# alshai/pfbwt-f

Measured on AMD Instinct MI355X. Metric: Gbases/s end-to-end BWT+SA build; bit-exact .bwt/.sa vs reference, higher is better.
Workload: dtype u8 text / u32 indices / u64 hash; 1 GPU; S-32G; L=32000000, H=1000, seed=1000, w=10, p=100, flags=-r, uint_t=64, n=32000010000, r=83625322, input=text resident in HBM, outputs (.bwt, .ssa, .esa) left in HBM, per_rank=single GPU

## Files before the change

pfbwt-f_amd/csrc/emit.h:

```cpp
#pragma once
#include "prims.h"
#include "parse.h"

namespace pfp {

__global__ __launch_bounds__(BLOCK) void k_pbwt_pack(const uint32_t *P, const uint8_t *last, const tpos_t *sai, uint64_t m, uint4 *rec)
{
    const uint64_t j = (uint64_t)blockIdx.x * BLOCK + threadIdx.x;
    if (j >= m) return;
    const uint64_t v = sai ? (uint64_t)sai[j] : 0ULL;
    rec[j] = make_uint4((uint32_t)v, (uint32_t)(v >> 32), P[j], (uint32_t)last[j ? j - 1 : m - 1]);
}
constexpr int BWL_SHIFT = 29;
__device__ __forceinline__ uint32_t bwl_code(uint32_t c) { return c == 0 ? 0u : c == Dollar ? 1u : c == '-' ? 2u : c == 'A' ? 3u : c == 'C' ? 4u : c == 'G' ? 5u : c == 'N' ? 6u : c == 'T' ? 7u : 8u; }
__device__ __forceinline__ uint8_t bwl_byte(uint32_t code) { return code == 0 ? (uint8_t)0 : code == 1 ? Dollar : code == 2 ? (uint8_t)'-' : code == 3 ? (uint8_t)'A' : code == 4 ? (uint8_t)'C' : code == 5 ? (uint8_t)'G' : code == 6 ? (uint8_t)'N' : (uint8_t)'T'; }
__global__ __launch_bounds__(BLOCK) void k_pbwt_rows(const uint32_t *SAP, const uint4 *rec, uint64_t m, uint8_t *bwlast, tpos_t *bwsai, uint32_t *W, uint32_t *rowid, int pack, uint32_t *bad)
{
    const uint64_t i = (uint64_t)blockIdx.x * BLOCK + threadIdx.x;
    if (i > m) return;
    const uint32_t s = SAP[i];
    if (s == 0) { bwlast[i] = 0; if (bwsai) bwsai[i] = 0; W[i] = 0; rowid[i] = (uint32_t)i; return; }
    const uint4 R = rec[s - 1];
    bwlast[i] = (uint8_t)R.w;
    if (bwsai) bwsai[i] = (tpos_t)(((uint64_t)R.y << 32) | R.x);
// ... 626 lines not shown

constexpr int EG_BUF = 4096, EG_PER_THREAD = EG_BUF / BLOCK;
constexpr int EG1_BUF = 8192, EG2_BUF = 16384;
__device__ __forceinline__ uint32_t group_members(const EmitArgs &a, const uint4 &S) { const uint32_t k = S.w & 0xFFFFFFu; return k == 0xFFFFFFu ? a.gk[S.z] : k; }
template <typename EBT> __global__ __launch_bounds__(BLOCK) void k_special_pack(EmitArgs a, uint32_t nsp, uint4 *cinfo, unsigned long long *cgb)
{
    const uint64_t j = (uint64_t)blockIdx.x * BLOCK + threadIdx.x;
    if (j >= nsp) return;
    const uint32_t i = a.elist[j]; const uint4 S = a.sinfo[i];
    const uint32_t fl = S.w >> 24; const bool multi = (fl & SF_MULTI) != 0;
    cinfo[j] = make_uint4(S.x, multi ? group_members(a, S) : 1u, multi ? i - S.z : 0u, (uint32_t)a.s_pc[i] | (fl << 8));
    cgb[j] = (unsigned long long)reinterpret_cast<const EBT *>(a.EB)[multi ? S.z : i];
}
template <typename EBT> __device__ __forceinline__ uint64_t group_start_at_or_after(const EBT *ENB, const uint4 *cinfo, uint64_t nsp, uint64_t lo, uint64_t v)
{
    while (lo < nsp && (uint64_t)ENB[lo] < v) ++lo;
    if (lo >= nsp) return nsp;
    const uint4 ci = cinfo[lo];
    if (!((ci.w >> 8) & SF_MULTI)) return lo;
    const uint64_t head = lo - ci.z;
    return (uint64_t)ENB[head] < v ? head + ci.y : head;
}
template <typename EBT> __global__ __launch_bounds__(BLOCK) void k_tile_own(const EBT *ENB, const uint4 *cinfo, const uint32_t *etile_slot, uint64_t nsp, uint64_t ntiles, uint32_t *town)
{
    const uint64_t t = (uint64_t)blockIdx.x * BLOCK + threadIdx.x;
    if (t > ntiles) return;
    town[t] = (uint32_t)group_start_at_or_after<EBT>(ENB, cinfo, nsp, etile_slot[t], t * EMIT_TILE);
}
template <typename EBT> __global__ __launch_bounds__(BLOCK) void k_emit_groups(EmitArgs a, uint8_t *bwt, uint32_t *qrow)
{
    __shared__ uint32_t LQ[EG_BUF];
    __shared__ uint32_t s_eb[EG_SLOTS + 1], s_fb[EG_SLOTS], s_kf[EG_SLOTS], s_dl[EG_SLOTS];
    __shared__ uint64_t s_ob[EG_SLOTS];
    __shared__ uint8_t s_pc[EG_SLOTS];
    __shared__ uint32_t red[4];
    __shared__ uint64_t jb[2];
    const EBT *ENB = reinterpret_cast<const EBT *>(a.ENB);
    const uint64_t tile0 = a.e0 / EMIT_TILE, tb = tile0 + blockIdx.x;
    const uint64_t o0 = tb * EMIT_TILE > a.e0 ? tb * EMIT_TILE : a.e0;
    const uint64_t o1 = ((tb + 1) * EMIT_TILE < a.e1) ? (tb + 1) * EMIT_TILE : a.e1;
    if (threadIdx.x < 2) {
        const uint64_t v = threadIdx.x ? o1 : o0;
        const uint64_t tv = threadIdx.x ? tb + 1 : tb;
        uint64_t j;
        if (v == tv * EMIT_TILE) j = a.town[tv];
        else {
            uint64_t lo = a.etile_slot[tb], hi = (uint64_t)a.etile_slot[tb + 1] + 1u;
            if (hi > a.ecount) hi = a.ecount;
            if (lo > hi) lo = hi;
            while (lo < hi) { const uint64_t mid = lo + ((hi - lo) >> 1); if ((uint64_t)ENB[mid] < v) lo = mid + 1; else hi = mid; }
            j = group_start_at_or_after<EBT>(ENB, a.cinfo, a.ecount, lo, v);
        }
        jb[threadIdx.x] = j;
    }
    __syncthreads();
    uint64_t j = jb[0]; const uint64_t jE = jb[1];
    const uint32_t cap = a.group_rows_cap < (uint32_t)EG_BUF ? a.group_rows_cap : (uint32_t)EG_BUF;
    while (j < jE) {
        const uint32_t nload = jE - j < (uint64_t)EG_SLOTS ? (uint32_t)(jE - j) : (uint32_t)EG_SLOTS;
        const uint64_t B0 = (uint64_t)ENB[j];
        uint32_t cand[2] = {0u, 0u}, bad = 0xFFFFFFFFu;
#pragma unroll
        for (int t = 0; t < 2; ++t) {
            const uint32_t s = threadIdx.x + (uint32_t)t * BLOCK;
            if (s < nload) {
                const uint4 ci = a.cinfo[j + s];
                const uint32_t fl = ci.w >> 8, dl = ci.z, k = ci.y;
                const uint64_t e0 = (uint64_t)ENB[j + s] - B0, e1 = (uint64_t)ENB[j + s + 1] - B0;
                s_eb[s] = e0 < 0xFFFFFFFFull ? (uint32_t)e0 : 0xFFFFFFFFu;
                if (s + 1 == nload) s_eb[nload] = e1 < 0xFFFFFFFFull ? (uint32_t)e1 : 0xFFFFFFFFu;
                s_fb[s] = ci.x; s_kf[s] = (k < 0xFFFFFFu ? k : 0xFFFFFFu) | (fl << 24); s_dl[s] = dl; s_pc[s] = (uint8_t)ci.w;
                s_ob[s] = (uint64_t)a.cgb[j + s];
                if (((fl & (SF_GFULL | SF_BIG)) || k > a.rank_members_max) && s < bad) bad = s;
                if (dl + 1u == k && e1 <= (uint64_t)cap) cand[t] = s + 1u;
            }
        }
        uint32_t tot;
        (void)block_incl_max(~bad, red, &tot);
        const uint32_t firstbad = ~tot;
        uint32_t c = 0;
#pragma unroll
        for (int t = 0; t < 2; ++t) if (cand[t] && cand[t] <= firstbad && cand[t] > c) c = cand[t];
        uint32_t cut;
        (void)block_incl_max(c, red, &cut);
        if (cut == 0) {
            const uint32_t k0 = a.cinfo[j].y;
            const uint64_t r0 = B0, r1 = (uint64_t)ENB[j + k0];
            {
                const uint32_t f0 = s_kf[0] >> 24;
                if (threadIdx.x == 0) {
                    unsigned long long idx = ~0ULL;
                    if (a.lglist && (f0 & SF_MULTI) && !(f0 & (SF_GFULL | SF_BIG)) && k0 <= (uint32_t)EG_SLOTS && r1 - r0 <= (uint64_t)EG2_BUF) {
                        const int big = r1 - r0 > (uint64_t)EG1_BUF ? 1 : 0;
                        idx = atomicAdd(a.lgcount + big, 1ULL);
                        if (idx < a.lgcap) a.lglist[(uint64_t)big * a.lgcap + idx] = (uint32_t)j;
                    }
                    jb[0] = idx < a.lgcap ? 1 : 0;
                }
                __syncthreads();
                const bool taken = jb[0] != 0;
                __syncthreads();
                if (taken) { j += k0; continue; }
            }
            if (threadIdx.x == 0) a.gleft[j] = 1;
            if (a.gstat && threadIdx.x == 0) {
                const uint32_t f0 = s_kf[0] >> 24;
                atomicAdd(&a.gstat[(f0 & SF_GFULL) ? 0 : (f0 & SF_BIG) ? 1 : (r1 - r0 > (uint64_t)cap) ? 2 : 3], (unsigned long long)(r1 - r0));
                int b = 0; while (b < 7 && (1024ull << (2 * b)) <= r1 - r0) ++b;
                atomicAdd(&a.gstat[4 + b], (unsigned long long)(r1 - r0));
            }
            if (r1 > r0) for (uint64_t t = r0 / EMIT_TILE + threadIdx.x; t <= (r1 - 1) / EMIT_TILE; t += BLOCK) a.tile_left[t - tile0] = 1;
            j += k0;
            __syncthreads();
            continue;
        }
        __syncthreads();
        const uint32_t nrows = s_eb[cut];
#pragma unroll
        for (int t = 0; t < 2; ++t) { const uint32_t s = threadIdx.x + (uint32_t)t * BLOCK; if (s < cut) s_ob[s] -= (uint64_t)s_eb[s - s_dl[s]]; }
        uint32_t qv[EG_PER_THREAD], sv[EG_PER_THREAD]; uint8_t cv[EG_PER_THREAD];
#pragma unroll
        for (int it = 0; it < EG_PER_THREAD; ++it) {
            const uint32_t r = threadIdx.x + (uint32_t)it * BLOCK;
            sv[it] = 0; qv[it] = 0; cv[it] = 0;
            if (r < nrows) {
                const uint32_t s = upper_bound_t<uint32_t>(s_eb, cut, r) - 1u, at = s_fb[s] + (r - s_eb[s]);
                sv[it] = s; qv[it] = a.ilist[at];
                if (!((s_kf[s] >> 24) & SF_MULTI) && a.bwl_il) cv[it] = a.bwl_il[at];
            }
        }
#pragma unroll
        for (int it = 0; it < EG_PER_THREAD; ++it) {
            const uint32_t r = threadIdx.x + (uint32_t)it * BLOCK;
            if (r < nrows) { LQ[r] = qv[it]; const uint32_t fl = s_kf[sv[it]] >> 24; if (fl & SF_MULTI) cv[it] = s_pc[sv[it]]; else if (!a.bwl_il) cv[it] = a.bwlast[qv[it]]; }
        }
        __syncthreads();
#pragma unroll
        for (int it = 0; it < EG_PER_THREAD; ++it) {
            const uint32_t r = threadIdx.x + (uint32_t)it * BLOCK;
            if (r < nrows) {
                const uint32_t s = sv[it], kf = s_kf[s];
                uint32_t pos = r;
                if ((kf >> 24) & SF_MULTI) {
                    const uint32_t sh = s - s_dl[s], k = kf & 0xFFFFFFu, q = qv[it];
                    uint32_t before = 0;
                    for (uint32_t mm = 0; mm < k; ++mm) {
                        const uint32_t sm = sh + mm;
                        if (sm != s) before += lower_bound_u32(LQ + s_eb[sm], s_eb[sm + 1] - s_eb[sm], q);
                    }
                    pos = s_eb[sh] + before + (r - s_eb[s]);
                }
                if (qrow) qrow[B0 - a.q0 + pos] = qv[it];
                const uint64_t o = s_ob[s] + pos;
                if (o >= a.w0 && o < a.w1) bwt[o - a.w0] = cv[it];
            }
        }
        __syncthreads();
        j += cut;
    }
}

template <int ITEMS> __device__ __forceinline__ void lds_sort_pairs_u32(uint32_t *keys, uint16_t *vals, uint32_t n, int npass, uint32_t (*wh)[RS_RADIX], uint32_t *red)
{
    const int lane = threadIdx.x & 63, wave = threadIdx.x >> 6;
    const uint32_t nit = (n + BLOCK - 1) / BLOCK;
    for (uint32_t j = n + threadIdx.x; j < nit * BLOCK; j += BLOCK) { keys[j] = 0xFFFFFFFFu; vals[j] = 0; }
    const uint32_t base = (uint32_t)wave * (nit * WAVE) + lane;
    for (int p = 0; p < npass; ++p) {
        const int sh = 8 * p;
        uint32_t k[ITEMS], dg[ITEMS]; uint16_t v[ITEMS];
#pragma unroll
        for (int w = 0; w < BLOCK / WAVE; ++w) wh[w][threadIdx.x] = 0;
        __syncthreads();
#pragma unroll
        for (int it = 0; it < ITEMS; ++it) {
            if ((uint32_t)it < nit) {
                const uint32_t i = base + (uint32_t)it * WAVE;
                k[it] = keys[i]; v[it] = vals[i];
                const uint32_t d = (k[it] >> sh) & 255u;
                uint32_t plo = 0xFFFFFFFFu, phi = 0xFFFFFFFFu;
                same_digit_lanes(d, plo, phi);
                const int leader = plo ? __builtin_ctz(plo) : 32 + __builtin_ctz(phi);
                uint32_t old = 0;
                if (lane == leader) { old = wh[wave][d]; wh[wave][d] = old + (uint32_t)__builtin_popcount(plo) + (uint32_t)__builtin_popcount(phi); }
                old = __shfl(old, leader);
                dg[it] = d | ((old + __builtin_amdgcn_mbcnt_hi(phi, __builtin_amdgcn_mbcnt_lo(plo, 0u))) << 8);
            }
        }
        __syncthreads();
        {
            const unsigned d = threadIdx.x;
            uint32_t cw[BLOCK / WAVE]; uint32_t total = 0;
#pragma unroll
            for (int w = 0; w < BLOCK / WAVE; ++w) { cw[w] = wh[w][d]; total += cw[w]; }
            uint32_t tt;
            uint32_t run = block_excl_sum(total, red, &tt);
#pragma unroll
            for (int w = 0; w < BLOCK / WAVE; ++w) { wh[w][d] = run; run += cw[w]; }
        }
        __syncthreads();
#pragma unroll
        for (int it = 0; it < ITEMS; ++it) {
            if ((uint32_t)it < nit) { const uint32_t li = wh[wave][dg[it] & 255u] + (dg[it] >> 8); keys[li] = k[it]; vals[li] = v[it]; }
        }
        __syncthreads();
    }
}
template <typename EBT, int BUF> __global__ __launch_bounds__(BLOCK) void k_emit_groups_large(EmitArgs a, uint8_t *bwt, uint32_t *qrow)
{
    __shared__ uint32_t LQ[BUF];
    __shared__ uint16_t LS[BUF];
    __shared__ uint32_t wh[BLOCK / WAVE][RS_RADIX];
    __shared__ uint32_t s_eb[EG_SLOTS + 1], s_fb[EG_SLOTS];
    __shared__ uint8_t s_pc[EG_SLOTS];
    __shared__ uint32_t red[4];
    const EBT *ENB = reinterpret_cast<const EBT *>(a.ENB);
    constexpr int WHICH = BUF > EG1_BUF ? 1 : 0;
    const unsigned long long have = a.lgcount[WHICH];
    const uint64_t cnt = have < a.lgcap ? have : a.lgcap;
    for (uint64_t g = blockIdx.x; g < cnt; g += gridDim.x) {
        const uint64_t j = a.lglist[(uint64_t)WHICH * a.lgcap + g];
        const uint32_t k = a.cinfo[j].y;
        const uint64_t B0 = (uint64_t)ENB[j], outbase = (uint64_t)a.cgb[j];
        for (uint32_t s = threadIdx.x; s < k; s += BLOCK) {
            const uint4 ci = a.cinfo[j + s];
            s_eb[s] = (uint32_t)((uint64_t)ENB[j + s] - B0); s_fb[s] = ci.x; s_pc[s] = (uint8_t)ci.w;
            if (s + 1 == k) s_eb[k] = (uint32_t)((uint64_t)ENB[j + k] - B0);
        }
        __syncthreads();
        const uint32_t nrows = s_eb[k];
        for (uint32_t r = threadIdx.x; r < nrows; r += BLOCK) { const uint32_t s = upper_bound_t<uint32_t>(s_eb, k, r) - 1u; LQ[r] = a.ilist[s_fb[s] + (r - s_eb[s])]; LS[r] = (uint16_t)s; }
        __syncthreads();
        lds_sort_pairs_u32<BUF / BLOCK>(LQ, LS, nrows, a.qpasses, wh, red);
        for (uint32_t r = threadIdx.x; r < nrows; r += BLOCK) {
            if (qrow) qrow[B0 - a.q0 + r] = LQ[r];
            const uint64_t o = outbase + r;
            if (o >= a.w0 && o < a.w1) bwt[o - a.w0] = s_pc[LS[r]];
        }
        __syncthreads();
    }
}

template <typename EBT> __global__ __launch_bounds__(BLOCK) void k_slice_bounds(EmitArgs a, uint64_t lo, uint64_t hi, unsigned long long *out)
{
    if (blockIdx.x != 0 || threadIdx.x != 0) return;
    const EBT *EB = reinterpret_cast<const EBT *>(a.EB);
    const EBT *ENB = reinterpret_cast<const EBT *>(a.ENB);
    const uint32_t il = slot_of_row<EBT>(a, lo);
    const uint32_t gh = (a.s_fl[il] & SF_MULTI) ? a.s_g0[il] : il;
    out[0] = EB[gh];
    out[2] = a.special ? (unsigned long long)ENB[a.cpos[gh]] : 0ULL;
    if (hi >= a.nout) { out[1] = a.nout; out[3] = a.special ? (unsigned long long)ENB[a.ecount] : 0ULL; return; }
    uint32_t s = slot_of_row<EBT>(a, hi - 1);
    if (a.s_fl[s] & SF_MULTI) { const uint32_t g = a.s_g0[s]; while (s < a.dsize && (a.s_fl[s] & SF_MULTI) && a.s_g0[s] == g) ++s; }
    else ++s;
    {
        uint64_t lo_ = s, hi_ = a.dsize;
        while (lo_ < hi_) { const uint64_t mid = lo_ + ((hi_ - lo_) >> 1); if ((uint64_t)EB[mid] < hi) lo_ = mid + 1; else hi_ = mid; }
        s = (uint32_t)lo_;
    }
    out[1] = s < a.dsize ? (uint64_t)EB[s] : a.nout;
    out[3] = a.special ? (unsigned long long)ENB[s < a.dsize ? a.cpos[s] : a.ecount] : 0ULL;
}

#ifndef PFP_FILL_NT
#define PFP_FILL_NT 0
#endif
__device__ __forceinline__ void fill_store16(uint8_t *dst, uint32_t x0, uint32_t x1, uint32_t x2, uint32_t x3)
{
#if PFP_FILL_NT && !defined(PFBWT_EMU_HIP_RUNTIME_H)
    typedef uint32_t fill_v4u __attribute__((ext_vector_type(4)));
    fill_v4u v = {x0, x1, x2, x3};
    __builtin_nontemporal_store(v, reinterpret_cast<fill_v4u *>(dst));
#else
    *reinterpret_cast<uint4 *>(dst) = make_uint4(x0, x1, x2, x3);
#endif
}
constexpr int FILL_PER_THREAD = 16, FILL_SUB = BLOCK * FILL_PER_THREAD;
constexpr int FILL_GROUPS = 4;
constexpr uint32_t FILL_MAX_SUBS = 8;
static_assert(FILL_SUB % EMIT_TILE == 0, "fill tiles are whole emission tiles");
template <typename EBT> __global__ __launch_bounds__(BLOCK) void k_fill(EmitArgs a, uint8_t *bwt, uint32_t subs_per_wg)
{
    __shared__ uint32_t eb[FILL_SUB + 2];
    __shared__ uint8_t pcs[FILL_SUB + 2];
    __shared__ uint32_t wcnt[BLOCK / WAVE];
    __shared__ uint32_t sts[FILL_MAX_SUBS * FILL_GROUPS + 1];
    const EBT *EB = reinterpret_cast<const EBT *>(a.EB);
    const EBT *cnt = reinterpret_cast<const EBT *>(a.cnt);
    const uint64_t ntiles = (a.nout + EMIT_TILE - 1) / EMIT_TILE;
    constexpr uint64_t TPS = FILL_SUB / EMIT_TILE;
    constexpr uint64_t SUPER = (uint64_t)FILL_GROUPS * FILL_SUB;
    const uint64_t st0 = a.w0 / SUPER + (uint64_t)blockIdx.x * subs_per_wg;
    const int lane = threadIdx.x & 63, wave = threadIdx.x >> 6;
    const unsigned long long lt = lane ? (~0ULL >> (64 - lane)) : 0ULL;
    for (uint32_t k = threadIdx.x; k <= subs_per_wg * FILL_GROUPS; k += BLOCK) {
        const uint64_t t = (st0 * FILL_GROUPS + k) * TPS;
        sts[k] = a.tile_slot[t < ntiles ? t : ntiles];
    }
    __syncthreads();
    auto compact = [&](uint32_t i0, uint32_t i1, uint64_t base) -> uint32_t {
        const uint32_t ns = i1 - i0 + 1u;
        uint32_t nz = 0;
        for (uint32_t k0 = 0; k0 < ns; k0 += BLOCK) {
            const uint32_t k = k0 + threadIdx.x;
            const EBT cn = k < ns ? cnt[i0 + k] : (EBT)0;
            const uint64_t e = k < ns ? (uint64_t)EB[i0 + k] : 0ULL;
            const uint8_t pc = k < ns ? a.s_pc[i0 + k] : (uint8_t)0;
            const bool has = cn != 0;
            const unsigned long long bal = __ballot(has);
            __syncthreads();
            if (lane == 0) wcnt[wave] = (uint32_t)__popcll(bal);
            __syncthreads();
            uint32_t pos = nz, tot = 0;
#pragma unroll
            for (int v = 0; v < BLOCK / WAVE; ++v) { const uint32_t cw = wcnt[v]; if (v < wave) pos += cw; tot += cw; }
            if (nz + tot > (uint32_t)FILL_SUB + 1u) return ~0u;
            if (has) { pos += (uint32_t)__popcll(bal & lt); eb[pos] = e > base ? (uint32_t)(e - base) : 0u; pcs[pos] = pc; }
            nz += tot;
        }
        if (threadIdx.x == 0) eb[nz] = 0xFFFFFFFFu;
        __syncthreads();
        return nz;
    };
    auto write_group = [&](uint64_t g0, uint64_t base, uint32_t nz) {
        const uint64_t o0 = g0 > a.w0 ? g0 : a.w0;
        const uint64_t o1 = g0 + FILL_SUB < a.w1 ? g0 + FILL_SUB : a.w1;
        const uint64_t ra = g0 + (uint64_t)threadIdx.x * FILL_PER_THREAD;
        const uint64_t lo = ra > o0 ? ra : o0, hi = ra + FILL_PER_THREAD < o1 ? ra + FILL_PER_THREAD : o1;
        if (lo >= hi) return;
        uint32_t wd[FILL_PER_THREAD / 4] = {0, 0, 0, 0};
        uint32_t rel = (uint32_t)(lo - base);
        uint32_t s = upper_bound_t<uint32_t>(eb, nz, rel) - 1u;
        uint32_t nxt = eb[s + 1], c = pcs[s];
        if (lo == ra && hi == ra + FILL_PER_THREAD && nxt >= rel + FILL_PER_THREAD) {
            wd[0] = wd[1] = wd[2] = wd[3] = c * 0x01010101u;
        } else {
#pragma unroll
            for (int j = 0; j < FILL_PER_THREAD; ++j) {
                const uint64_t o = ra + j;
                if (o >= lo && o < hi) {
                    while (rel >= nxt) { ++s; nxt = eb[s + 1]; c = pcs[s]; }
                    wd[j >> 2] |= c << (8 * (j & 3));
                    ++rel;
                }
            }
        }
        uint8_t *dst = bwt + (ra - a.w0);
        if (lo == ra && hi == ra + FILL_PER_THREAD) fill_store16(dst, wd[0], wd[1], wd[2], wd[3]);
        else for (uint64_t o = lo; o < hi; ++o) { const int j = (int)(o - ra); dst[j] = (uint8_t)(wd[j >> 2] >> (8 * (j & 3))); }
    };
    for (uint32_t ss = 0; ss < subs_per_wg; ++ss) {
        const uint64_t tstart = (st0 + ss) * SUPER;
        if (tstart >= a.w1) break;
        const uint64_t tend = tstart + SUPER < a.w1 ? tstart + SUPER : a.w1;
        const uint32_t ng = (uint32_t)((tend - tstart + FILL_SUB - 1) / FILL_SUB);
        const uint32_t *gs = sts + ss * FILL_GROUPS;
        uint32_t nz = compact(gs[0], gs[ng], tstart);
        if (nz != ~0u) {
            for (uint32_t g = 0; g < ng; ++g) write_group(tstart + (uint64_t)g * FILL_SUB, tstart, nz);
        } else {
            for (uint32_t g = 0; g < ng; ++g) {
                const uint64_t g0 = tstart + (uint64_t)g * FILL_SUB;
                nz = compact(gs[g], gs[g + 1], g0);
                write_group(g0, g0, nz);
            }
        }
    }
}

__global__ __launch_bounds__(BLOCK) void k_run_count(const uint8_t *bwt, uint64_t nout, int has_prev, unsigned long long *runs)
{
    __shared__ uint32_t red[4];
    const uint64_t o0 = ((uint64_t)blockIdx.x * BLOCK + threadIdx.x) * 16;
    uint32_t cntr = 0;
    if (o0 < nout) {
        uint8_t prev = (o0 || has_prev) ? *(bwt + o0 - 1) : (uint8_t)0;
        for (int k = 0; k < 16 && o0 + k < nout; ++k) { const uint8_t cc = bwt[o0 + k]; cntr += cc != prev; prev = cc; }
    }
    uint32_t tot;
    (void)block_excl_sum(cntr, red, &tot);
    if (threadIdx.x == 0 && tot) atomicAdd(runs, (unsigned long long)tot);
}
constexpr int RUN_PER_THREAD = 16, RUN_TILE = BLOCK * RUN_PER_THREAD;
__device__ __forceinline__ uint32_t run_mask16(const uint8_t *bwt, uint64_t j0, uint64_t rows, int has_prev)
{
    if (j0 >= rows) return 0;
    const uint64_t lo = ld8(bwt + j0), hi = ld8(bwt + j0 + 8);
    const uint64_t prev = (j0 || has_prev) ? (uint64_t)*(bwt + j0 - 1) : 0ULL;
    const uint64_t xl = lo ^ ((lo << 8) | prev), xh = hi ^ ((hi << 8) | (lo >> 56));
    uint32_t m = 0;
#pragma unroll
    for (int b = 0; b < 8; ++b) { m |= ((xl >> (8 * b)) & 0xff) ? (1u << b) : 0u; m |= ((xh >> (8 * b)) & 0xff) ? (1u << (8 + b)) : 0u; }
    const uint64_t left = rows - j0;
    return left >= 16 ? m : (m & ((1u << left) - 1u));
}
__global__ __launch_bounds__(BLOCK) void k_run_tile_count(const uint8_t *bwt, uint64_t rows, int has_prev, uint32_t *tilecnt, uint16_t *rmask)
{
    __shared__ uint32_t red[4];
    const uint64_t g = (uint64_t)blockIdx.x * BLOCK + threadIdx.x;
    const uint32_t m = run_mask16(bwt, g * RUN_PER_THREAD, rows, has_prev);
    if (rmask) rmask[g] = (uint16_t)m;
    uint32_t tot;
    (void)block_excl_sum((uint32_t)__popc(m), red, &tot);
    if (threadIdx.x == 0) tilecnt[blockIdx.x] = tot;
}
constexpr int SR_TILES = 8;
template <typename SAT> __global__ __launch_bounds__(BLOCK) void k_sample_rows(const uint16_t *rmask, uint64_t rows, uint64_t ntiles, const uint32_t *tilebase, uint64_t row_base, uint64_t run_base, uint64_t total_rows,
                                                                               uint64_t total_runs_plus1 , SAT *ssa, SAT *esa)
{
    __shared__ unsigned long long red[4];
    const uint64_t t0 = (uint64_t)blockIdx.x * SR_TILES;
    uint32_t m[SR_TILES]; unsigned long long c[2] = {0ULL, 0ULL};
#pragma unroll
    for (int b = 0; b < SR_TILES; ++b) {
        const uint64_t g = (t0 + b) * BLOCK + threadIdx.x;
        m[b] = (t0 + b < ntiles && g * RUN_PER_THREAD < rows) ? (uint32_t)rmask[g] : 0u;
        c[b >> 2] |= (unsigned long long)__popc(m[b]) << (16 * (b & 3));
    }
    unsigned long long tot;
    const unsigned long long e0 = block_excl_sum(c[0], red, &tot), e1 = block_excl_sum(c[1], red, &tot);
#pragma unroll
    for (int b = 0; b < SR_TILES; ++b) {
        if (t0 + b >= ntiles) break;
        const uint64_t j0 = ((t0 + b) * BLOCK + threadIdx.x) * RUN_PER_THREAD;
        uint32_t mm = m[b];
        uint64_t k = run_base + tilebase[t0 + b] + (uint32_t)(((b < 4 ? e0 : e1) >> (16 * (b & 3))) & 0xFFFFu);
        while (mm) {
            const int bit = __ffs((int)mm) - 1; mm &= mm - 1;
            const uint64_t o = row_base + j0 + bit;
            ssa[2 * k] = (SAT)o;
            if (o) esa[2 * (k - 1)] = (SAT)(o - 1);
            ++k;
        }
        if (total_runs_plus1 && j0 < rows && row_base + rows == total_rows && total_rows - 1 - row_base - j0 < RUN_PER_THREAD)
            *(esa + 2 * ((long long)total_runs_plus1 - 2)) = (SAT)(total_rows - 1);
    }
}
template <typename SAT, typename EBT> __global__ __launch_bounds__(BLOCK) void k_sample_values(EmitArgs a, const SAT *sa_win, const uint32_t *qrow, uint64_t w_first, uint64_t rc, uint64_t run_base,
                                                                                               int has_last, uint64_t last_idx, SAT *ssa, SAT *esa)
{
    const EBT *EB = reinterpret_cast<const EBT *>(a.EB);
    auto value = [&](uint64_t o) -> SAT {
        if (sa_win) return sa_win[o - w_first];
        if (o == 0) return (SAT)a.n;
        const uint32_t slot = slot_of_row<EBT>(a, o);
        uint32_t q;
        if (!a.special) q = qrow[o - w_first];
        else {
            const uint4 S = a.sinfo[slot]; const uint32_t fl = S.w >> 24;
            if (slot_is_special(fl)) {
                const uint32_t g = (fl & SF_MULTI) ? S.z : slot;
                q = a.qspec[(uint64_t)reinterpret_cast<const EBT *>(a.ENB)[a.cpos[g]] - a.q0 + (o - (uint64_t)EB[g])];
            } else if (!(fl & SF_MULTI)) q = a.ilist[S.x + (uint32_t)(o - (uint64_t)EB[slot])];
            else q = (o == (uint64_t)EB[S.z]) ? a.gqf[S.z] : a.gql[S.z];
        }
        return (SAT)((SAT)a.bwsai[q] - (SAT)a.s_sl[slot]);
    };
    const uint64_t i = (uint64_t)blockIdx.x * BLOCK + threadIdx.x;
    if (i < rc) {
        const uint64_t k = run_base + i;
        const uint64_t o = (uint64_t)ssa[2 * k];
        ssa[2 * k + 1] = value(o);
        if (o) esa[2 * (k - 1) + 1] = value(o - 1);
    } else if (i == rc && has_last) *(esa + 2 * (long long)last_idx + 1) = value(a.nout - 1);
}

}
```

Before: 124.2 Gbases/s.

## Prefetch compaction loads, hint run search, fill runs wordwise, compact whole workgroup span

The BWT fill kernel now software-prefetches the next block's count/boundary/char loads during compaction. It keeps a per-thread search hint so each group's upper_bound starts from the previous run index. It also writes runs into two 64-bit words with shifts instead of a per-byte loop. Finally, it first tries to compact the entire workgroup span at once and falls back to the per-supertile path only if the span overflows the shared buffer. Together these aim to cut memory latency, repeated binary searches and per-byte work in the emission stage, at the cost of extra register pressure and more complex control flow.

Result: no change. 124.9 Gbases/s, median of 6 (+0.6%).

```diff
diff --git a/pfbwt-f_amd/csrc/emit.h b/pfbwt-f_amd/csrc/emit.h
--- a/pfbwt-f_amd/csrc/emit.h
+++ b/pfbwt-f_amd/csrc/emit.h
@@ -952,11 +952,16 @@
     auto compact = [&](uint32_t i0, uint32_t i1, uint64_t base) -> uint32_t {
         const uint32_t ns = i1 - i0 + 1u;
         uint32_t nz = 0;
+        auto gather = [&](uint32_t k, EBT &cn, uint64_t &e, uint8_t &pc) {
+            const uint32_t i = i0 + (k < ns ? k : 0u);
+            cn = cnt[i]; e = (uint64_t)EB[i]; pc = a.s_pc[i];
+            if (k >= ns) cn = (EBT)0;
+        };
+        EBT ncn; uint64_t ne; uint8_t npc;
+        gather(threadIdx.x, ncn, ne, npc);
         for (uint32_t k0 = 0; k0 < ns; k0 += BLOCK) {
-            const uint32_t k = k0 + threadIdx.x;
-            const EBT cn = k < ns ? cnt[i0 + k] : (EBT)0;
-            const uint64_t e = k < ns ? (uint64_t)EB[i0 + k] : 0ULL;
-            const uint8_t pc = k < ns ? a.s_pc[i0 + k] : (uint8_t)0;
+            const EBT cn = ncn; const uint64_t e = ne; const uint8_t pc = npc;
+            if (k0 + BLOCK < ns) gather(k0 + BLOCK + threadIdx.x, ncn, ne, npc);
             const bool has = cn != 0;
             const unsigned long long bal = __ballot(has);
             __syncthreads();
@@ -973,33 +978,53 @@
         __syncthreads();
         return nz;
     };
-    auto write_group = [&](uint64_t g0, uint64_t base, uint32_t nz) {
+    auto write_group = [&](uint64_t g0, uint64_t base, uint32_t nz, uint32_t &shint) {
         const uint64_t o0 = g0 > a.w0 ? g0 : a.w0;
         const uint64_t o1 = g0 + FILL_SUB < a.w1 ? g0 + FILL_SUB : a.w1;
         const uint64_t ra = g0 + (uint64_t)threadIdx.x * FILL_PER_THREAD;
         const uint64_t lo = ra > o0 ? ra : o0, hi = ra + FILL_PER_THREAD < o1 ? ra + FILL_PER_THREAD : o1;
         if (lo >= hi) return;
         uint32_t wd[FILL_PER_THREAD / 4] = {0, 0, 0, 0};
-        uint32_t rel = (uint32_t)(lo - base);
-        uint32_t s = upper_bound_t<uint32_t>(eb, nz, rel) - 1u;
+        const uint32_t rel = (uint32_t)(lo - base);
+        uint32_t s = shint + upper_bound_t<uint32_t>(eb + shint, nz - shint, rel) - 1u;
+        shint = s;
         uint32_t nxt = eb[s + 1], c = pcs[s];
         if (lo == ra && hi == ra + FILL_PER_THREAD && nxt >= rel + FILL_PER_THREAD) {
             wd[0] = wd[1] = wd[2] = wd[3] = c * 0x01010101u;
         } else {
-#pragma unroll
-            for (int j = 0; j < FILL_PER_THREAD; ++j) {
-                const uint64_t o = ra + j;
-                if (o >= lo && o < hi) {
-                    while (rel >= nxt) { ++s; nxt = eb[s + 1]; c = pcs[s]; }
-                    wd[j >> 2] |= c << (8 * (j & 3));
-                    ++rel;
+            const uint32_t relA = (uint32_t)(ra - base), je = (uint32_t)(hi - ra);
+            uint64_t h0 = 0, h1 = 0;
+            uint32_t j = (uint32_t)(lo - ra);
+            for (;;) {
+                uint32_t end = nxt - relA;
+                if (end > je) end = je;
+                if (end > j) {
+                    const uint64_t v = (uint64_t)c * 0x0101010101010101ULL;
+                    if (j < 8) { const uint32_t e = end < 8 ? end : 8; h0 |= (v >> (64 - 8 * (e - j))) << (8 * j); }
+                    if (end > 8) { const uint32_t b = j > 8 ? j : 8; h1 |= (v >> (64 - 8 * (end - b))) << (8 * (b - 8)); }
+                    j = end;
                 }
-            }
+                if (j >= je) break;
+                ++s; nxt = eb[s + 1]; c = pcs[s];
+            }
+            wd[0] = (uint32_t)h0; wd[1] = (uint32_t)(h0 >> 32); wd[2] = (uint32_t)h1; wd[3] = (uint32_t)(h1 >> 32);
         }
         uint8_t *dst = bwt + (ra - a.w0);
         if (lo == ra && hi == ra + FILL_PER_THREAD) fill_store16(dst, wd[0], wd[1], wd[2], wd[3]);
         else for (uint64_t o = lo; o < hi; ++o) { const int j = (int)(o - ra); dst[j] = (uint8_t)(wd[j >> 2] >> (8 * (j & 3))); }
     };
+    {
+        const uint64_t wstart = st0 * SUPER;
+        if (wstart >= a.w1) return;
+        const uint64_t wend = wstart + (uint64_t)subs_per_wg * SUPER < a.w1 ? wstart + (uint64_t)subs_per_wg * SUPER : a.w1;
+        const uint32_t ng = (uint32_t)((wend - wstart + FILL_SUB - 1) / FILL_SUB);
+        const uint32_t nz = compact(sts[0], sts[ng], wstart);
+        if (nz != ~0u) {
+            uint32_t sh = 0;
+            for (uint32_t g = 0; g < ng; ++g) write_group(wstart + (uint64_t)g * FILL_SUB, wstart, nz, sh);
+            return;
+        }
+    }
     for (uint32_t ss = 0; ss < subs_per_wg; ++ss) {
         const uint64_t tstart = (st0 + ss) * SUPER;
         if (tstart >= a.w1) break;
@@ -1008,12 +1033,14 @@
         const uint32_t *gs = sts + ss * FILL_GROUPS;
         uint32_t nz = compact(gs[0], gs[ng], tstart);
         if (nz != ~0u) {
-            for (uint32_t g = 0; g < ng; ++g) write_group(tstart + (uint64_t)g * FILL_SUB, tstart, nz);
+            uint32_t sh = 0;
+            for (uint32_t g = 0; g < ng; ++g) write_group(tstart + (uint64_t)g * FILL_SUB, tstart, nz, sh);
         } else {
             for (uint32_t g = 0; g < ng; ++g) {
                 const uint64_t g0 = tstart + (uint64_t)g * FILL_SUB;
                 nz = compact(gs[g], gs[g + 1], g0);
-                write_group(g0, g0, nz);
+                uint32_t sh = 0;
+                write_group(g0, g0, nz, sh);
             }
         }
     }
```
